# Nicolas-Zamorano/pytorch_fem_solver

Hardware: AMD Instinct MI355X
Metric: Melements/s assembled (global K + f) (higher is better)
Workload: dtype f64

## Files before the change

### pytorch_fem_solver_amd/basis/engine.py

```python

from __future__ import annotations

import ctypes
import math
import os
from ctypes import c_void_p

import numpy as np
import torch

from .. import _native
from ..sparse import CSRMatrix


class NoDeviceError(RuntimeError):
    pass


def _is_block(u):
    return u is not None and u.dim() == 2 and u.shape[1] > 1


def _compute_device(home: torch.device) -> torch.device:
    if home.type == "cuda":
# ... 155 lines not shown
                c_void_p(coords.ctypes.data), c_void_p(rowptr.ctypes.data),
                c_void_p(colind.ctypes.data), own_cap, vert_cap, flags, ctypes.byref(handle),
                ctypes.byref(n_priority),
            )
        )
    try:
        layout = np.zeros(32, dtype=np.int64)
        _native.check(lib.tfem_ring_plan_sizes(handle, c_void_p(layout.ctypes.data)))
        blob = np.empty(int(layout[12]), dtype=np.uint8)
        _native.check(lib.tfem_ring_plan_pack(handle, c_void_p(blob.ctypes.data)))
    finally:
        lib.tfem_ring_plan_destroy(handle)
    plan = unpack_ring_plan(blob, layout)
    plan["n_priority"] = int(n_priority.value)
    return plan


def unpack_ring_plan(blob, layout):
    z = [int(x) for x in layout]

    def view(i, dtype, count):
        return np.frombuffer(blob, dtype=dtype, count=count, offset=z[8 + i])

    return {
        "blob": blob,
        "layout": np.ascontiguousarray(layout, dtype=np.int64),
        "n_tiles": z[0],
        "slots": z[6],
        "words": z[7],
        "chunked": bool(z[13]),
        "desc": view(0, np.int32, 20 * z[0]),
        "rows": view(1, np.uint32, z[7] * z[1]),
        "rowstart": view(2, np.int32, z[1]),
        "vert_gid": view(3, np.int32, z[2]),
        "row_ecodes": np.frombuffer(blob, dtype=np.uint32, count=((12 * z[6] + 31) // 32) * z[1], offset=z[15]),
        "tile_elems": np.frombuffer(blob, dtype=np.int32, count=z[19], offset=z[16]),
        "tile_tverts": np.frombuffer(blob, dtype=np.uint32, count=z[21], offset=z[20]),
        "long_rows": np.frombuffer(blob, dtype=np.uint32, count=24 * z[23], offset=z[22]),
        "elems_staged": bool(z[18]),
        "chain_order": np.frombuffer(blob, dtype=np.int32, count=z[0], offset=z[24]),
        "chain_len": z[25],
        "hand_in": np.frombuffer(blob, dtype=np.uint16, count=z[1], offset=z[26]),
        "max_n_tv": z[27],
        "n_runs": z[28],
        "runs": np.frombuffer(blob, dtype=np.int32, count=(z[28] + 1 if z[28] > 0 else 0), offset=z[30]),
    }


def p2_plan_host(conn_dof, n_verts, n_dofs, coords, rowptr, colind):
    lib = _native.load()
    conn = np.ascontiguousarray(np.asarray(conn_dof).astype(np.int32)).reshape(-1, 6)
    coords = np.ascontiguousarray(np.asarray(coords, dtype=np.float64)).reshape(-1, 2)
    rowptr = np.ascontiguousarray(np.asarray(rowptr, dtype=np.int64))
    colind = np.ascontiguousarray(np.asarray(colind, dtype=np.int32))
    handle = c_void_p()
    _native.check(
        lib.tfem_p2_plan_create(
            c_void_p(conn.ctypes.data), conn.shape[0], int(n_verts), int(n_dofs),
            c_void_p(coords.ctypes.data), c_void_p(rowptr.ctypes.data),
            c_void_p(colind.ctypes.data), ctypes.byref(handle),
        )
    )
    try:
        layout = np.zeros(24, dtype=np.int64)
        _native.check(lib.tfem_p2_plan_sizes(handle, c_void_p(layout.ctypes.data)))
        blob = np.zeros(int(layout[16]), dtype=np.uint8)
        _native.check(lib.tfem_p2_plan_pack(handle, c_void_p(blob.ctypes.data)))
    finally:
# ... 424 lines not shown
            return {"priority": (0, p), "rest": (p, n - p), "all": (0, n)}[which]
        except KeyError:
            raise ValueError(f"tiles: {which!r} is not 'priority', 'rest' or 'all'") from None

    def _resident_source_workgroups(self):
        cus = 256
        if self.device.type == "cuda":
            cus = int(torch.cuda.get_device_properties(self.device).multi_processor_count)
        try:
            reserve = max(0, int(os.environ.get("TFEM_RINGS_RESERVE_CUS", "0") or 0))
        except ValueError:
            reserve = 0
        return (max(8, cus - 8 * reserve) * 4 // 8) * 8

    def ring_plan(self):
        if self._rings is None:
            self._rings = False
            if self.kernel in ("auto", "rings") and self._p1_plan_eligible():
                self.csr_structure()
                rowptr, colind = self._csr_host
                wgs_given = os.environ.get("TFEM_RING_WGS")
                if wgs_given is None:
                    os.environ["TFEM_RING_WGS"] = str(self._resident_source_workgroups())
                try:
                    plan = ring_plan_host(
                        self._conn_host_np(), self.n_dofs, self._coords_host_np(), rowptr, colind,
                        priority=self._priority_vertices, pattern=self._pattern,
                    )
                except NotImplementedError:
                    plan = None
                finally:
                    if wgs_given is None:
                        os.environ.pop("TFEM_RING_WGS", None)
                    if self._pattern is not None:
                        self._pattern.release()
                        self._pattern = None
                if plan is not None:
                    step = np.diff(plan["rowstart"].astype(np.int64))
                    n_runs = 1 + int(np.count_nonzero((step <= 0) | (step > 16)))
                    self._rings = {
                        "blob": torch.from_numpy(plan["blob"]).to(self.device),
                        "layout": plan["layout"],
                        "chunked": plan["chunked"],
                        "elems_staged": plan["elems_staged"],
                        "has_tverts": int(plan["layout"][21]) > 0 or int(plan["layout"][19]) == 0,
                        "fq_ok": bool(plan["elems_staged"]) and int(plan["layout"][23]) == 0,
                        "rows_per_run": plan["rowstart"].size / n_runs,
                        "n_tiles": plan["n_tiles"],
                        "n_priority": plan["n_priority"],
                    }
            if self._rings is False and self.kernel == "rings":
                raise NotImplementedError("the ring-plan kernel does not apply to this basis")
        return self._rings or None

    def p2_plan(self):
        if self._p2rows is None:
# ... 967 lines not shown
```

### pytorch_fem_solver_amd/csrc/tfem_rings.hip

```cpp
#include <cmath>

#include "tfem_rings_kernel.hpp"

namespace tfem {

template <typename T, bool MASS>
__global__ __launch_bounds__(kRingBlock) void k_p1_long_rows(const T *coords, const unsigned char *plan,
                                                             unsigned off_long, int n_long, T *vals, T stiff_w,
                                                             T mass_d, T mass_o) {
  RingLongSlot<T> s;
  ring_long_slot<T, MASS, false>(coords, plan, off_long, n_long, stiff_w, mass_o, nullptr, s);
  if (!s.slot) return;
  T *out = vals + s.rec[1];
  out[int((s.rec[19 + s.i / 8] >> (4 * (s.i % 8))) & 15u)] = s.entry;
  if (s.i == 0) out[s.dpos] = ring_diag<T, MASS>(s.sum, s.dsum, mass_d, mass_o);
}

struct RingLaunch {
  const void *coords;
  int quad_order;
  double alpha, beta;
  const unsigned char *plan;
  const int64_t *layout;
  int64_t n_verts, nnz;
// ... 190 lines not shown
    a.u_first = int(t_first);
    if (z[28] > 0 && (t_first != 0 || t_count != z[0]))
      return fail(TFEM_ERR_UNSUPPORTED, "tile ranges need a plan built with flagged vertices (its blocks break between the ranges)");
    if (z[28] > 0) {
      a.n_runs = int(z[28]);
      a.off_runs = unsigned(z[30]);
    }
  } else {
    a.off_desc += 80u * unsigned(t_first);
  }
  const bool mass = L.beta != 0.0;
  const int slots = int(z[6]);
  a.lds_elem = load ? int(z[17]) : 0;
  const size_t lds = size_t(4 * a.lds_vert) * sizeof(T) +
                     (kmat ? size_t(kRingWaves) * size_t(64 * (slots + 1) + 2) * sizeof(T) : 0) +
                     (src ? size_t(3 * (a.lds_vert + 2)) * sizeof(T)
                          : load ? size_t(3 * a.lds_elem + 4) * sizeof(T) : 0);
  const bool chunk = z[13] != 0;
  a.plain_stores = !load;
  if (const char *v = std::getenv("TFEM_RINGS_STORES")) a.plain_stores = std::strcmp(v, "plain") == 0;
  const bool wide = src && ring_src_wide(L.source);
  const bool separable = src && ring_src_route<T>(z, L.coords, tables.nq, L.source) == 2;
  if (separable) ring_separable_weights<T>(L.source, a.qsym);
  void *kernel = pick_ring_kernel<T>(slots, mass, chunk, load ? tables.nq : 0, src, kmat, wide, separable);
  if (!kernel) return fail(TFEM_ERR_UNSUPPORTED, "Integration order not implemented");
  int per_cu = 0;
  st = resident_per_cu(kernel, kRingBlock, lds, &per_cu);
  if (st != TFEM_OK) return st;
  const int deal = a.xcd_interleave > 0 ? a.xcd_interleave : 1;
  int per = int((t_count + 8 * deal - 1) / (8 * deal)) * deal;
  if (src) {
    const int64_t first_block = t_first / a.chain_len, last_block = (t_first + t_count - 1) / a.chain_len;
    per = int((last_block - first_block + 1 + 7) / 8);
    if (a.n_runs > 0) per = (a.n_runs + 7) / 8;
  }
  if (L.blocks_per_cu > 0 && L.blocks_per_cu < per_cu) per_cu = L.blocks_per_cu;
  int cus = device_cu_count();
  if (const char *v = std::getenv("TFEM_RINGS_RESERVE_CUS")) cus = std::max(8, cus - 8 * std::max(0, std::atoi(v)));
  const int blocks = std::min(per * 8, (cus * per_cu / 8) * 8);
  const dim3 grid{unsigned(blocks)}, block{unsigned(kRingBlock)};
  void *params[] = {&a};
  hipError_t e = hipLaunchKernel(kernel, grid, block, params, lds, L.stream);
  if (e != hipSuccess) return fail(TFEM_ERR_HIP, "ring kernel launch: %s", hipGetErrorString(e));
  if (kmat && z[23] > 0) {
    const dim3 lgrid{unsigned((16 * z[23] + kRingBlock - 1) / kRingBlock)};
    if (mass)
// ... 117 lines not shown
```

### pytorch_fem_solver_amd/csrc/tfem_rings_host.cpp

```cpp
#include <algorithm>
#include <cmath>
#include <cstdlib>
#include <cstring>
#include <memory>
#include <numeric>
#include <vector>
#include <chrono>
#include <cstdio>

#include "tfem_common.hpp"
#include "tfem_threads.hpp"

namespace tfem {

constexpr int kRingDescStride = 20;
constexpr int kRingLayoutLen = 32;
constexpr int kRingElemCap = 768;
constexpr int kRingElemRuns = 8;
constexpr int kRingHaloCapHost = 256;

struct RingPlan {
  int slots = 7, words = 4;
  std::vector<int32_t> desc;
  std::vector<uint32_t> rows;
  std::vector<int32_t> rowstart;
  std::vector<int32_t> tile_elems;
  std::vector<uint32_t> row_ecodes;
  std::vector<uint32_t> tile_tverts;
  std::vector<uint32_t> long_rows;
  int32_t max_n_elem = 0;
  bool elems_staged = true;
  std::vector<int32_t> vert_gid;
  int32_t max_n_vert = 0, max_n_own = 0, max_row_len = 0, max_n_halo = 0;
  int64_t n_tiles = 0;
  bool chunked = false;
  bool long_mode = false;
  int64_t n_priority = 0;
  std::vector<int32_t> chain_order;
  std::vector<uint16_t> hand_in;
  int32_t chain_len = 1;
  std::vector<int32_t> runs;
  int32_t chain_wgs = 1024;
  int32_t max_n_tv = 0;
};

namespace {

inline uint64_t ring_spread_bits(uint64_t x) {
  x &= 0xFFFFFFFFull;
  x = (x | (x << 16)) & 0x0000FFFF0000FFFFull;
  x = (x | (x << 8)) & 0x00FF00FF00FF00FFull;
  x = (x | (x << 4)) & 0x0F0F0F0F0F0F0F0Full;
  x = (x | (x << 2)) & 0x3333333333333333ull;
  x = (x | (x << 1)) & 0x5555555555555555ull;
  return x;
}

struct Fan {
  int k = 0;
  int32_t nb[16];
  int flag[16];
  int32_t elem[16];
  int loc[16];
};

// ... 495 lines not shown
  std::vector<uint8_t> starts(size_t(n_tiles), 0);
  if (runs.empty()) {
    for (int64_t u = 0; u < n_tiles; u += len) starts[size_t(u)] = 1;
    if (n_priority > 0 && n_priority < n_tiles) starts[size_t(n_priority)] = 1;
    return starts;
  }
  for (size_t w = 0; w + 1 < runs.size(); ++w)
    if (runs[w] < runs[w + 1]) starts[size_t(runs[w])] = 1;
  return starts;
}

void chain_pass(const std::vector<TileSpec> &specs, RingPlan &plan) {
  const int64_t n_tiles = plan.n_tiles;
  plan.chain_order.resize(size_t(n_tiles));
  std::iota(plan.chain_order.begin(), plan.chain_order.end(), 0);
  auto by_curve = [&](int32_t x, int32_t y) { return specs[size_t(x)].curve_rank < specs[size_t(y)].curve_rank; };
  std::sort(plan.chain_order.begin(), plan.chain_order.begin() + plan.n_priority, by_curve);
  std::sort(plan.chain_order.begin() + plan.n_priority, plan.chain_order.end(), by_curve);
  const int len = pick_chain_len(n_tiles);
  plan.chain_len = len;
  plan.chain_wgs = 1024;
  if (const char *v = std::getenv("TFEM_RING_WGS")) plan.chain_wgs = std::max(8, std::atoi(v));
  plan.runs.clear();
  bool use_runs = plan.n_priority == 0;
  if (const char *v = std::getenv("TFEM_RING_RUNS")) use_runs = use_runs && std::atoi(v) != 0;
  if (use_runs) plan.runs = chain_runs(n_tiles, plan.chain_wgs);
  const std::vector<uint8_t> starts = chain_block_starts(n_tiles, len, plan.runs, plan.n_priority);
  plan.hand_in.assign(plan.rowstart.size(), uint16_t(0xFFFF));
  std::vector<int64_t> block_first;
  for (int64_t u = 0; u < n_tiles; ++u)
    if (starts[size_t(u)]) block_first.push_back(u);
  block_first.push_back(n_tiles);
  const int64_t n_blocks = int64_t(block_first.size()) - 1;
  std::vector<std::vector<uint32_t>> kept(static_cast<size_t>(n_tiles));
  int32_t *desc = plan.desc.data();
  auto elem_id = [&](const int32_t *d, int32_t j) {
    const int32_t *te = plan.tile_elems.data() + d[16];
    if (!d[18]) return te[j];
    int32_t id = te[0] + j;
    for (int r = 1; r < kRingElemRuns; ++r)
      if (j >= te[kRingElemRuns + r - 1]) id = te[r] + (j - te[kRingElemRuns + r - 1]);
    return id;
  };
  parallel_for(n_blocks, [&](int64_t b0, int64_t b1, int) {
    TileMap prev(16384), cur(16384), prev_local(2048);
    for (int64_t b = b0; b < b1; ++b) {
// ... 287 lines not shown
          return fail(TFEM_ERR_UNSUPPORTED, "vertex %d alone exceeds the tile capacity", u);
        break;
      }
      for (int32_t w : fresh) vert_stamp[size_t(w)] = tile;
      n_local += int(fresh.size());
      spec.owned.push_back(u);
      ++cursor;
    }
    std::sort(spec.owned.begin(), spec.owned.end());
    for (int w = 0; w < 5; ++w) spec.wave_start[w] = std::min<int32_t>(64 * w, int32_t(spec.owned.size()));
    spec.curve_rank = tile;
    specs.push_back(std::move(spec));
    ++tile;
  }
  lap("greedy tiling along the curve");
  priority_first(specs);
  const int st = emit_plan(conn, adj_ptr_data, adj_data, rowptr, colind, elem_ranges, specs, plan);
  lap("emitting tiles");
  if (st == TFEM_OK) chain_pass(specs, plan);
  lap("chain order, element tables");
  return st;
}

void ring_layout(const RingPlan &p, int64_t layout[kRingLayoutLen]) {
  std::memset(layout, 0, sizeof(int64_t) * kRingLayoutLen);
  layout[0] = p.n_tiles;
  layout[1] = int64_t(p.rowstart.size());
  layout[2] = int64_t(p.vert_gid.size());
  layout[3] = p.max_n_vert;
  layout[4] = p.max_n_own;
  layout[5] = p.max_row_len;
  layout[6] = p.slots;
  layout[7] = p.words;
  const int64_t bytes[11] = {int64_t(p.desc.size()) * 4, int64_t(p.rows.size()) * 4,
                             int64_t(p.rowstart.size()) * 4, int64_t(p.vert_gid.size()) * 4,
                             int64_t(p.row_ecodes.size()) * 4, int64_t(p.tile_elems.size()) * 4,
                             int64_t(p.tile_tverts.size()) * 4, int64_t(p.long_rows.size()) * 4,
                             int64_t(p.chain_order.size()) * 4, int64_t(p.hand_in.size()) * 2,
                             int64_t(p.runs.size()) * 4};
  const int slot_of[11] = {8, 9, 10, 11, 15, 16, 20, 22, 24, 26, 30};
  int64_t off = 0;
  for (int i = 0; i < 11; ++i) {
    layout[slot_of[i]] = off;
    off += (bytes[i] + 15) & ~int64_t(15);
  }
  layout[12] = off + 64;
  layout[17] = p.max_n_elem;
  layout[18] = p.elems_staged ? 1 : 0;
  layout[19] = int64_t(p.tile_elems.size());
  layout[21] = int64_t(p.tile_tverts.size());
  layout[23] = int64_t(p.long_rows.size() / 24);
  layout[13] = p.chunked ? 1 : 0;
  layout[14] = p.max_n_halo;
  layout[25] = p.chain_len;
  layout[27] = p.max_n_tv;
  layout[28] = p.runs.empty() ? -1 : p.chain_wgs;
}

}
}

namespace tfem {
namespace {
int ring_plan_build(const void *conn_host, int idx_bytes, int64_t n_elems, int64_t n_verts,
                    const double *coords_host, const int64_t *rowptr_host, const int32_t *colind_host,
                    int own_cap, int vert_cap, const uint8_t *vertex_priority_host, const int64_t *inc_ptr,
                    int32_t *inc, void **plan_out, int64_t *n_priority_tiles) {
  if (!plan_out) return fail(TFEM_ERR_INVALID_ARGUMENT, "plan_out is NULL");
// ... 75 lines not shown
  auto *out = static_cast<unsigned char *>(blob_host);
  struct Part { int64_t off; const void *src; int64_t bytes; };
  const Part parts[11] = {
      {layout[8], p->desc.data(), int64_t(p->desc.size()) * 4},
      {layout[9], p->rows.data(), int64_t(p->rows.size()) * 4},
      {layout[10], p->rowstart.data(), int64_t(p->rowstart.size()) * 4},
      {layout[11], p->vert_gid.data(), int64_t(p->vert_gid.size()) * 4},
      {layout[15], p->row_ecodes.data(), int64_t(p->row_ecodes.size()) * 4},
      {layout[16], p->tile_elems.data(), int64_t(p->tile_elems.size()) * 4},
      {layout[20], p->tile_tverts.data(), int64_t(p->tile_tverts.size()) * 4},
      {layout[22], p->long_rows.data(), int64_t(p->long_rows.size()) * 4},
      {layout[24], p->chain_order.data(), int64_t(p->chain_order.size()) * 4},
      {layout[26], p->hand_in.data(), int64_t(p->hand_in.size()) * 2},
      {layout[30], p->runs.data(), int64_t(p->runs.size()) * 4},
  };
  for (const Part &part : parts) {
    const int64_t padded = (part.bytes + 15) & ~int64_t(15);
    std::memset(out + part.off + part.bytes, 0, size_t(padded - part.bytes));
    if (part.bytes == 0) continue;
    parallel_for(part.bytes, [&](int64_t b, int64_t e, int) {
      std::memcpy(out + part.off + b, static_cast<const unsigned char *>(part.src) + b, size_t(e - b));
    }, 1 << 20);
  }
  std::memset(out + layout[12] - 64, 0, 64);
  return TFEM_OK;
}

int tfem_ring_plan_vouch_coords(int64_t *plan_layout_host, const void *coords, double max_abs_coord) {
  if (!plan_layout_host) return tfem::fail(TFEM_ERR_INVALID_ARGUMENT, "plan_layout_host is NULL");
  int64_t bits = 0, array = 0;
  if (coords && max_abs_coord >= 0.0 && std::isfinite(max_abs_coord)) {
    std::memcpy(&bits, &max_abs_coord, sizeof(bits));
    array = int64_t(reinterpret_cast<uintptr_t>(coords));
  }
  plan_layout_host[29] = array;
  plan_layout_host[31] = bits;
  return TFEM_OK;
}

void tfem_ring_plan_destroy(void *plan_handle) { delete static_cast<tfem::RingPlan *>(plan_handle); }

}
```

### pytorch_fem_solver_amd/csrc/tfem_rings_kernel.hpp

```cpp
#pragma once

#include <hip/hip_runtime.h>

#include <algorithm>
#include <cstdlib>
#include <cstring>
#include <type_traits>

#include "tfem_common.hpp"
#include "tfem_rowkit.hpp"
#include "tfem_source.hpp"

#pragma clang fp contract(fast)

namespace tfem {

constexpr int kRingBlock = 256;
constexpr int kRingWaves = kRingBlock / 64;
constexpr int kRingVertCap = 1024;

template <typename T>
struct RingArgs {
  const T *coords;
  const unsigned char *plan;
// ... 379 lines not shown
}

template <int SLOTS>
__device__ __forceinline__ void ring_load_rec(ring_rsrc_t r, unsigned byte, RingRec<SLOTS> &rec) {
  const ru32x4 v = __builtin_amdgcn_raw_buffer_load_b128(r, byte, 0, kStreamLoadNT);
  rec.w[0] = v.x;
  rec.w[1] = v.y;
  rec.w[2] = v.z;
  rec.w[3] = v.w;
  if constexpr (SLOTS == 15) {
    const ru32x4 u = __builtin_amdgcn_raw_buffer_load_b128(r, byte + 16u, 0, kStreamLoadNT);
    rec.w[4] = u.x;
    rec.w[5] = u.y;
    rec.w[6] = u.z;
    rec.w[7] = u.w;
  }
}

struct RingDesc {
  int vert_off, n_vert, row_off, n_own, row0, row1, gid0, rs0, elem_off, n_elem, elem_mode, tvert_off;
  int n_tv;
};
constexpr int kRingElemRuns = 8;

template <bool CHUNK>
__device__ __forceinline__ RingDesc ring_desc(const unsigned char *plan, unsigned off_desc, int tile,
                                              int wave) {
  ring_const_i32 d = (ring_const_i32)(uintptr_t)(plan + off_desc + 80u * unsigned(tile));
  RingDesc r{d[0], d[1], d[2], d[7], d[3 + wave], d[4 + wave], 0, 0, d[16], d[17], d[18] & 0xFF, d[19], d[18] >> 8};
  if (CHUNK) {
    r.gid0 = d[8 + wave];
    r.rs0 = d[12 + wave];
  }
  return r;
}

constexpr int kRingHaloCap = kRingBlock;
constexpr int kRingElemPerLane = 3;

__device__ __forceinline__ void ring_lds_barrier() {
  asm volatile("s_waitcnt lgkmcnt(0)\n\ts_barrier" ::: "memory");
}

constexpr int kFqLoadNT = 0;
template <typename T, int QL>
__device__ __forceinline__ void ring_load_fq(ring_rsrc_t r, unsigned byte, T (&v)[QL > 0 ? QL : 1]) {
// ... 89 lines not shown
    }
  };
  ring_rsrc_t r_coords = ring_rsrc(a.coords, a.coords_bytes);
  ring_rsrc_t r_plan = ring_rsrc(a.plan, a.plan_bytes);
  ring_rsrc_t r_vals = ring_rsrc(a.vals, a.vals_bytes);
  const ring_rsrc_t r_fq = ring_rsrc(a.fq, a.fq_bytes);
  ring_rsrc_t r_fout = ring_rsrc(a.fout, a.fout_bytes);
  constexpr unsigned kRecBytes = unsigned(4 * RingRec<SLOTS>::kWords);
  constexpr unsigned kNone = 0x3FFFFFFu;
  auto tile_rsrc = [&](unsigned off, int first, int count, int size) {
    const unsigned at = off + unsigned(first * size);
    const int room = int(plan_room - at), want = count * size;
    const int fits = want < room ? want : room;
    return ring_rsrc(plan_at + at, unsigned(fits > 0 ? fits : 0));
  };
  auto run_rsrc = [&](T *vals, unsigned vals_room, int first, int count) {
    const int at = first > 0 ? first : 0;
    const int room = int(vals_room / unsigned(sizeof(T))) - at;
    const int fits = count < room ? count : room;
    return ring_rsrc(reinterpret_cast<unsigned char *>(vals) + unsigned(at) * unsigned(sizeof(T)),
                     unsigned(fits > 0 ? fits : 0) * unsigned(sizeof(T)));
  };
  const unsigned lane_b2 = unsigned(lane) * 2u, lane_b4 = unsigned(lane) * 4u, lane_b16 = unsigned(lane) * 16u;
  if (FQ && tid < 4)
    gtab[3 * a.lds_elem + tid] = T(0);
  const int acc_stride = a.lds_vert + 2;
  T *accs = gtab;
  if (SRC)
    for (int i = tid; i < 3 * acc_stride; i += kRingBlock) accs[i] = T(0);

  SrcLanes<T> prog;
  if constexpr (SRC && !SEP) prog = src_load_lanes<T>(src_in_kernarg<T>(__builtin_offsetof(RingArgs<T>, src)));
  int sep_flags = 0;
  if constexpr (SEP) sep_flags = src_separable_flags<T>(src_in_kernarg<T>(__builtin_offsetof(RingArgs<T>, src)));
  RingRec<SLOTS> rec, rec_ld;
  uint32_t se[FQ ? kEW : 1], se_ld[FQ ? kEW : 1];
  unsigned eid[FQ ? kRingElemPerLane : 1], eid_ld[FQ ? kRingElemPerLane : 1];
  T fqe_ld[FQ ? kRingElemPerLane : 1][QL > 0 ? QL : 1];
  unsigned tev[SRC ? kRingElemPerLane : 1], tev_ld[SRC ? kRingElemPerLane : 1];
  unsigned gid_row = 0;
  int rowstart = 0, rowstart_ld = 0;
  unsigned gid_own = 0, gid_halo = 0;
  unsigned gid_own_ld = 0, gid_halo_ld = 0;
  T own_ld[2], halo_ld[2];
  unsigned hin = 0xFFFFu, hin_ld = 0xFFFFu;

// ... 161 lines not shown
        const T base = src_fma<T>(qs[0], f4[0], qs[1] * ((f4[1] + f4[2]) + f4[3]));
        share[j][0] = det * src_fma<T>(qs[2], f4[3], base);
        share[j][1] = det * src_fma<T>(qs[2], f4[1], base);
        share[j][2] = det * src_fma<T>(qs[2], f4[2], base);
      } else {
        T fw[QL > 0 ? QL : 1];
#pragma unroll
        for (int q = 0; q < QL; ++q) fw[q] = fv[j * (QL > 0 ? QL : 1) + q] * hwq[q];
#pragma unroll
        for (int i = 0; i < 3; ++i) {
          T g = T(0);
#pragma unroll
          for (int q = 0; q < QL; ++q) g = g + fw[q] * lamq[i][q];
          share[j][i] = det * g;
        }
      }
    }
#pragma unroll
    for (int j = 0; j < kNE; ++j)
#pragma unroll
      for (int i = 0; i < 3; ++i) asm volatile("" : "+v"(share[j][i]));
#pragma unroll
    for (int j = 0; j < kNE; ++j) {
      if (vtid + j * kRingBlock < d.n_tv) {
#pragma unroll
        for (int i = 0; i < 3; ++i) add_share((codes[j] >> (10 * i)) & 0x3FFu, acc, share[j][i]);
      }
    }
  };
  auto compute_g = [&](const RingDesc &d, const unsigned (&tv)[SRC ? kRingElemPerLane : 1], const T *xyc,
                       T *acc, int rot) {
    const int vwave = (wave + rot) & (kRingWaves - 1);
    const int vtid = (vwave << 6) + lane;
    const int rounds = (d.n_tv - vwave * 64 + kRingBlock - 1) / kRingBlock;
    if (rounds <= 0) return;
    if constexpr (SRC == 2) {
      if (rounds >= 3)
        compute_g_wide(std::integral_constant<int, 3>{}, d, tv, xyc, acc, vtid);
      else
        compute_g_wide(std::integral_constant<int, 2>{}, d, tv, xyc, acc, vtid);
    } else if constexpr (SRC == 1) {
      unsigned codes[kRingElemPerLane];
#pragma unroll
      for (int j = 0; j < kRingElemPerLane; ++j) codes[j] = tv[SRC ? j : 0];
#pragma unroll 1
      for (int j = 0; j < kRingElemPerLane; ++j) {
        if (j >= rounds) break;
        const int l = vtid + j * kRingBlock;
        const unsigned code = codes[0];
#pragma unroll
        for (int r = 0; r + 1 < kRingElemPerLane; ++r) codes[r] = codes[r + 1];
        T x0, y0, x1, y1, x2, y2;
        lds_xy(xyc, code & 0x3FFu, x0, y0);
        lds_xy(xyc, (code >> 10) & 0x3FFu, x1, y1);
// ... 62 lines not shown
      dst[2 * r + 1] = own_ld[1];
    }
    const int h = d.n_own + tid;
    if (h < d.n_vert) {
      dst[2 * h] = halo_ld[0];
      dst[2 * h + 1] = halo_ld[1];
    }
  };
  auto load_xy_lds = [&](const RingDesc &d, unsigned g_own, unsigned g_halo, T *dst) {
    if constexpr (kCoordsToLds) {
      typedef __attribute__((address_space(3))) void *lds_ptr;
      if constexpr (kTileDesc && CHUNK) {
        if (lane < d.row1 - d.row0)
          __builtin_amdgcn_raw_ptr_buffer_load_lds(r_coords, (lds_ptr)(dst + 2 * d.row0), 16,
                                                   (unsigned(lane) << 4) + unsigned(d.gid0) * 16u, 0, 0, 0);
      } else if (d.row0 + lane < d.row1)
        __builtin_amdgcn_raw_ptr_buffer_load_lds(r_coords, (lds_ptr)(dst + 2 * d.row0), 16, g_own * 16u, 0, 0, 0);
      if (d.n_own + tid < d.n_vert)
        __builtin_amdgcn_raw_ptr_buffer_load_lds(r_coords, (lds_ptr)(dst + 2 * (d.n_own + 64 * wave)), 16,
                                                 g_halo * 16u, 0, 0, 0);
    }
  };

  int t_c = tile_at(0);
  if (t_c < 0) return;
  int t_n = tile_at(1), t_nn = tile_at(2);
  RingDesc dc = ring_desc<CHUNK>(a.plan, a.off_desc, t_c, wave);
  RingDesc dn = ring_desc<CHUNK>(a.plan, a.off_desc, t_n >= 0 ? t_n : t_c, wave);
  RingDesc dnn = ring_desc<CHUNK>(a.plan, a.off_desc, t_nn >= 0 ? t_nn : t_c, wave);
  load_ids(dc, gid_own, gid_halo);
  load_eids(dc, eid);
  __builtin_amdgcn_s_waitcnt(0x0F70);
  load_tile(dc, gid_own, gid_halo);
  load_xy_lds(dc, gid_own, gid_halo, xy);
  load_fq(dc, eid);
  load_tverts(dc, tev_ld, 0);
  if (t_n >= 0) {
    load_ids(dn, gid_own_ld, gid_halo_ld);
    load_eids(dn, eid_ld);
  }
  __builtin_amdgcn_s_waitcnt(0x0F70);
  park(dc, xy);
  park_g(dc, gtab);
  rec = rec_ld;
  hin = hin_ld;
  rowstart = rowstart_ld;
  gid_row = gid_own;
#pragma unroll
  for (int i = 0; i < (FQ ? kEW : 1); ++i) se[i] = se_ld[i];
#pragma unroll
  for (int j = 0; j < (FQ ? kRingElemPerLane : 1); ++j) eid[j] = eid_ld[j];
#pragma unroll
  for (int j = 0; j < (SRC ? kRingElemPerLane : 1); ++j) tev[j] = tev_ld[j];
  gid_own = gid_own_ld;
  gid_halo = gid_halo_ld;
  __syncthreads();

  int cur = 0;
  int a_cur = 0, a_prev = 2, a_next = 1;
  for (int k = 0;; ++k) {
    if (SRC) {
      switch ((k + int(blockIdx.x >> kRingPrioShift)) & 3) {
        case 0: __builtin_amdgcn_s_setprio(0); break;
        case 1: __builtin_amdgcn_s_setprio(1); break;
        case 2: __builtin_amdgcn_s_setprio(2); break;
        default: __builtin_amdgcn_s_setprio(3); break;
      }
    }
    auto phase_a = [&]() {
      if (t_n >= 0) {
        load_tile(dn, gid_own, gid_halo);
        load_fq(dn, eid);
        load_tverts(dn, tev_ld, k + 1);
        if (t_nn >= 0) {
          load_ids(dnn, gid_own_ld, gid_halo_ld);
          load_eids(dnn, eid_ld);
        }
      }
    };
    if (SRC) {
      if (t_n >= 0) load_xy_lds(dn, gid_own, gid_halo, xy + (cur ^ 1) * 2 * a.lds_vert);
      compute_g(dc, tev, xy + cur * 2 * a.lds_vert, accs + a_cur * acc_stride, k);
      if constexpr (SEP) {
        typedef const RingArgs<T> __attribute__((address_space(4))) *ring_kernargs;
        const ring_kernargs ka = (ring_kernargs)src_kernarg_table<char>(0);
        r_coords = ring_rsrc(ka->coords, ka->coords_bytes);
        plan_at = ka->plan;
        plan_room = ka->plan_bytes;
        vals_at = ka->vals;
        vals_room = ka->vals_bytes;
        plain_now = ka->plain_stores;
        r_vals = ring_rsrc(vals_at, vals_room);
        r_fout = ring_rsrc(ka->fout, ka->fout_bytes);
      }
    }
    phase_a();
    T off[SLOTS + 1], diag, sdets[SLOTS];
    constexpr int kBandSlots = (SLOTS > kRingBand && kRingBand > 0) ? kRingBand : (SLOTS == 7 && SRC ? 6 : SLOTS);
    const bool banded = kBandSlots < SLOTS && __builtin_amdgcn_ballot_w64(rec.k() > kBandSlots) == 0;
    bool regular = false;
    const int my_row = dc.row0 + lane;
    const uint32_t lv = unsigned(my_row < dc.row1 ? my_row : 0);
    if constexpr (SLOTS == 7 && SRC) {
      const bool mine = ((rec.w[2] >> 10) & 0x3FFFu) == 0x555u && rec.k() == 6;
// ... 96 lines not shown
        __builtin_amdgcn_raw_buffer_store_b64(__builtin_bit_cast(ru32x2, facc), r_fout, byte, 0, kStreamNT);
      else
        __builtin_amdgcn_raw_buffer_store_b32(__builtin_bit_cast(unsigned, facc), r_fout, byte, 0, kStreamNT);
    }
    if (t_n < 0) break;
    rec = rec_ld;
    hin = hin_ld;
    rowstart = rowstart_ld;
    gid_row = gid_own;
#pragma unroll
    for (int i = 0; i < (FQ ? kEW : 1); ++i) se[i] = se_ld[i];
#pragma unroll
    for (int j = 0; j < (FQ ? kRingElemPerLane : 1); ++j) eid[j] = eid_ld[j];
#pragma unroll
    for (int j = 0; j < (SRC ? kRingElemPerLane : 1); ++j) tev[j] = tev_ld[j];
    gid_own = gid_own_ld;
    gid_halo = gid_halo_ld;
    {
      const int t = a_prev;
      a_prev = a_cur;
      a_cur = a_next;
      a_next = t;
    }
    ring_lds_barrier();
    t_c = t_n;
    dc = dn;
    t_n = t_nn;
    dn = dnn;
    t_nn = tile_at(k + 3);
    if (t_nn >= 0) dnn = ring_desc<CHUNK>(plan_now(), a.off_desc, t_nn, wave);
    cur ^= 1;
  }
}

template <typename T>
void *pick_ring_src_kernel(int slots, bool mass, bool chunk, int nq, bool kmat, bool wide, bool separable);
inline bool ring_src_runs_wide(int nq, bool wide) { return wide && nq <= 4; }

template <typename T>
static int ring_args_init(const TriTables &tables, const int64_t *z, const void *coords, const unsigned char *plan,
                   int64_t n_verts, double alpha, double beta, RingArgs<T> &a) {
  if (z[0] < 0 || z[4] > kRingBlock || z[3] > kRingVertCap || z[4] > z[3] || z[14] > kRingHaloCap ||
      !((z[6] == 7 && z[7] == 4) || (z[6] == 15 && z[7] == 8)) || (z[5] > z[6] + 1 && z[23] == 0) || z[5] > 16)
    return fail(TFEM_ERR_INVALID_ARGUMENT, "ring plan exceeds the kernel's capacities");
  const int64_t extents[2] = {n_verts * 2 * int64_t(sizeof(T)), z[12]};
  const int st = check_extents("ring kernel", extents, 2);
// ... 26 lines not shown
```

Measured before the change: 78190.

## Precompute per-wave tile walk records on host for separable source ring kernel

```diff
diff --git a/pytorch_fem_solver_amd/basis/engine.py b/pytorch_fem_solver_amd/basis/engine.py
--- a/pytorch_fem_solver_amd/basis/engine.py
+++ b/pytorch_fem_solver_amd/basis/engine.py
@@ -201,6 +201,8 @@
     def view(i, dtype, count):
         return np.frombuffer(blob, dtype=dtype, count=count, offset=z[8 + i])
 
+    has_walk = (bool(z[13]) and z[6] == 7 and z[28] > 0
+                and ((z[30] + 4 * (z[28] + 1) + 63) & ~63) + 256 * z[0] + 64 <= z[12])
     return {
         "blob": blob,
         "layout": np.ascontiguousarray(layout, dtype=np.int64),
@@ -223,6 +225,8 @@
         "max_n_tv": z[27],
         "n_runs": z[28],
         "runs": np.frombuffer(blob, dtype=np.int32, count=(z[28] + 1 if z[28] > 0 else 0), offset=z[30]),
+        "walk": np.frombuffer(blob, dtype=np.int32, count=(64 * z[0] if has_walk else 0),
+                              offset=(((z[30] + 4 * (z[28] + 1) + 63) & ~63) if has_walk else 0)).reshape(-1, 4, 16),
     }
 
 
@@ -693,6 +697,9 @@
                 wgs_given = os.environ.get("TFEM_RING_WGS")
                 if wgs_given is None:
                     os.environ["TFEM_RING_WGS"] = str(self._resident_source_workgroups())
+                walk_given = os.environ.get("TFEM_RING_WALK")
+                if walk_given is None:
+                    os.environ["TFEM_RING_WALK"] = "1"
                 try:
                     plan = ring_plan_host(
                         self._conn_host_np(), self.n_dofs, self._coords_host_np(), rowptr, colind,
@@ -703,6 +710,8 @@
                 finally:
                     if wgs_given is None:
                         os.environ.pop("TFEM_RING_WGS", None)
+                    if walk_given is None:
+                        os.environ.pop("TFEM_RING_WALK", None)
                     if self._pattern is not None:
                         self._pattern.release()
                         self._pattern = None
diff --git a/pytorch_fem_solver_amd/csrc/tfem_rings.hip b/pytorch_fem_solver_amd/csrc/tfem_rings.hip
--- a/pytorch_fem_solver_amd/csrc/tfem_rings.hip
+++ b/pytorch_fem_solver_amd/csrc/tfem_rings.hip
@@ -236,6 +236,11 @@
   const bool wide = src && ring_src_wide(L.source);
   const bool separable = src && ring_src_route<T>(z, L.coords, tables.nq, L.source) == 2;
   if (separable) ring_separable_weights<T>(L.source, a.qsym);
+  if (src) a.off_telems = 0;
+  if (separable && chunk && slots == 7 && a.n_runs > 0) {
+    const int64_t walk_at = (z[30] + 4 * (z[28] + 1) + 63) & ~int64_t(63);
+    if (walk_at + 256 * z[0] + 64 <= z[12]) a.off_telems = unsigned(walk_at);
+  }
   void *kernel = pick_ring_kernel<T>(slots, mass, chunk, load ? tables.nq : 0, src, kmat, wide, separable);
   if (!kernel) return fail(TFEM_ERR_UNSUPPORTED, "Integration order not implemented");
   int per_cu = 0;
diff --git a/pytorch_fem_solver_amd/csrc/tfem_rings_host.cpp b/pytorch_fem_solver_amd/csrc/tfem_rings_host.cpp
--- a/pytorch_fem_solver_amd/csrc/tfem_rings_host.cpp
+++ b/pytorch_fem_solver_amd/csrc/tfem_rings_host.cpp
@@ -41,6 +41,7 @@
   int32_t chain_len = 1;
   std::vector<int32_t> runs;
   int32_t chain_wgs = 1024;
+  bool with_walk = false;
   int32_t max_n_tv = 0;
 };
 
@@ -582,6 +583,7 @@
   plan.chain_wgs = 1024;
   if (const char *v = std::getenv("TFEM_RING_WGS")) plan.chain_wgs = std::max(8, std::atoi(v));
   plan.runs.clear();
+  if (const char *v = std::getenv("TFEM_RING_WALK")) plan.with_walk = v[0] == '1';
   bool use_runs = plan.n_priority == 0;
   if (const char *v = std::getenv("TFEM_RING_RUNS")) use_runs = use_runs && std::atoi(v) != 0;
   if (use_runs) plan.runs = chain_runs(n_tiles, plan.chain_wgs);
@@ -915,6 +917,43 @@
   return st;
 }
 
+constexpr int64_t kRingWalkBytes = 64;
+inline bool ring_has_walk(const RingPlan &p) { return p.with_walk && p.chunked && p.slots == 7 && !p.runs.empty(); }
+inline int64_t ring_walk_offset(int64_t off_runs, int64_t n_runs) { return (off_runs + 4 * (n_runs + 1) + 63) & ~int64_t(63); }
+
+void ring_walk_fill(const RingPlan &p, const int64_t *layout, int32_t *out) {
+  const int64_t n_runs = int64_t(p.runs.size()) - 1;
+  parallel_for(n_runs, [&](int64_t b, int64_t e, int) {
+    for (int64_t r = b; r < e; ++r)
+      for (int64_t u = p.runs[size_t(r)]; u < p.runs[size_t(r) + 1]; ++u) {
+        const int32_t *d = p.desc.data() + size_t(p.chain_order[size_t(u)]) * kRingDescStride;
+        const int64_t k = u - p.runs[size_t(r)];
+        for (int w = 0; w < 4; ++w) {
+          int32_t *rec = out + (size_t(u) * 4 + size_t(w)) * 16;
+          auto stream = [&](int at, int64_t section, int64_t first, int64_t count, int64_t size) {
+            rec[at] = int32_t(count > 0 ? section + first * size : section);
+            rec[at + 1] = int32_t(count > 0 ? count * size : 0);
+          };
+          const int64_t row0 = d[3 + w], rows = d[4 + w] - d[3 + w];
+          stream(0, layout[9], d[2] + row0, rows, 4 * p.words);
+          stream(2, layout[26], d[2] + row0, rows, 2);
+          const int64_t first_e = ((w + k) & 3) << 6, left = (d[18] >> 8) - first_e;
+          stream(4, layout[20], d[19] + first_e, left, 4);
+          rec[6] = int32_t(left);
+          rec[7] = int32_t(left > 0 ? (left + 255) / 256 : 0);
+          rec[8] = d[8 + w];
+          rec[9] = d[12 + w];
+          rec[10] = int32_t(row0);
+          rec[11] = int32_t(rows);
+          const int64_t halo0 = d[7] + 64 * w;
+          stream(12, layout[11], d[0] + halo0, d[1] - halo0, 4);
+          rec[14] = int32_t(halo0);
+          rec[15] = u + 1 == p.runs[size_t(r) + 1] ? 1 : 0;
+        }
+      }
+  }, 4);
+}
+
 void ring_layout(const RingPlan &p, int64_t layout[kRingLayoutLen]) {
   std::memset(layout, 0, sizeof(int64_t) * kRingLayoutLen);
   layout[0] = p.n_tiles;
@@ -937,6 +976,7 @@
     layout[slot_of[i]] = off;
     off += (bytes[i] + 15) & ~int64_t(15);
   }
+  if (ring_has_walk(p)) off = ring_walk_offset(layout[30], int64_t(p.runs.size()) - 1) + p.n_tiles * 4 * kRingWalkBytes;
   layout[12] = off + 64;
   layout[17] = p.max_n_elem;
   layout[18] = p.elems_staged ? 1 : 0;
@@ -1058,6 +1098,12 @@
       std::memcpy(out + part.off + b, static_cast<const unsigned char *>(part.src) + b, size_t(e - b));
     }, 1 << 20);
   }
+  if (ring_has_walk(*p)) {
+    const int64_t runs_end = layout[30] + ((int64_t(p->runs.size()) * 4 + 15) & ~int64_t(15));
+    const int64_t at = ring_walk_offset(layout[30], int64_t(p->runs.size()) - 1);
+    std::memset(out + runs_end, 0, size_t(at - runs_end));
+    ring_walk_fill(*p, layout, reinterpret_cast<int32_t *>(out + at));
+  }
   std::memset(out + layout[12] - 64, 0, 64);
   return TFEM_OK;
 }
diff --git a/pytorch_fem_solver_amd/csrc/tfem_rings_kernel.hpp b/pytorch_fem_solver_amd/csrc/tfem_rings_kernel.hpp
--- a/pytorch_fem_solver_amd/csrc/tfem_rings_kernel.hpp
+++ b/pytorch_fem_solver_amd/csrc/tfem_rings_kernel.hpp
@@ -425,6 +425,14 @@
   int n_tv;
 };
 constexpr int kRingElemRuns = 8;
+
+typedef int ring_walk_t __attribute__((ext_vector_type(16)));
+typedef int ring_walk_half_t __attribute__((ext_vector_type(8)));
+typedef int ring_walk_halo_t __attribute__((ext_vector_type(4)));
+enum : int {
+  kWalkRecOff = 0, kWalkRecBytes, kWalkHinOff, kWalkHinBytes, kWalkTvOff, kWalkTvBytes, kWalkTvLeft, kWalkRounds,
+  kWalkGid0, kWalkRs0, kWalkRow0, kWalkRows, kWalkHaloOff, kWalkHaloBytes, kWalkHaloSlot, kWalkLast
+};
 
 template <bool CHUNK>
 __device__ __forceinline__ RingDesc ring_desc(const unsigned char *plan, unsigned off_desc, int tile,
@@ -560,6 +568,94 @@
                      unsigned(fits > 0 ? fits : 0) * unsigned(sizeof(T)));
   };
   const unsigned lane_b2 = unsigned(lane) * 2u, lane_b4 = unsigned(lane) * 4u, lane_b16 = unsigned(lane) * 16u;
+  constexpr bool kWalk = kTileDesc && CHUNK && SLOTS == 7;
+  int n_gid0 = 0, n_rs0 = 0, n_row0 = 0, n_rows = 0, n_hbytes = 0, n_hslot = 0;
+  int hnn_off = 0, hnn_bytes = 0, hnn_last = 0, cur_left = 0, cur_rounds = 0;
+  unsigned wpos = 0, wpos_n = 0;
+  auto walking = [&]() {
+    unsigned at = a.off_telems;
+    asm volatile("" : "+s"(at));
+    return at != 0u;
+  };
+  auto walk_set_next = [&](const ring_walk_t &w) {
+    n_gid0 = w[kWalkGid0];
+    n_rs0 = w[kWalkRs0];
+    n_row0 = w[kWalkRow0];
+    n_rows = w[kWalkRows];
+    n_hbytes = w[kWalkHaloBytes];
+    n_hslot = w[kWalkHaloSlot];
+  };
+  auto walk_load_next = [&](unsigned at) {
+    typedef int pair_t __attribute__((ext_vector_type(2)));
+    typedef const pair_t __attribute__((address_space(4))) *pair_ptr;
+    const pair_t g = *(pair_ptr)(uintptr_t)(plan_now() + at + 4u * unsigned(kWalkGid0));
+    const pair_t r = *(pair_ptr)(uintptr_t)(plan_now() + at + 4u * unsigned(kWalkRow0));
+    const pair_t h = *(pair_ptr)(uintptr_t)(plan_now() + at + 4u * unsigned(kWalkHaloBytes));
+    n_gid0 = g[0];
+    n_rs0 = g[1];
+    n_row0 = r[0];
+    n_rows = r[1];
+    n_hbytes = h[0];
+    n_hslot = h[1];
+  };
+  auto walk_load = [&](unsigned at) {
+    typedef const ring_walk_t __attribute__((address_space(4))) *walk_ptr;
+    return *(walk_ptr)(uintptr_t)(plan_now() + at);
+  };
+  auto walk_load_half = [&](unsigned at) {
+    typedef const ring_walk_half_t __attribute__((address_space(4))) *half_ptr;
+    return *(half_ptr)(uintptr_t)(plan_now() + at);
+  };
+  auto walk_first = [&](const ring_walk_t &w) { return __builtin_shufflevector(w, w, 0, 1, 2, 3, 4, 5, 6, 7); };
+  auto walk_load_halo = [&](unsigned at) {
+    typedef const ring_walk_halo_t __attribute__((address_space(4))) *halo_ptr;
+    const ring_walk_halo_t h = *(halo_ptr)(uintptr_t)(plan_now() + at + 4u * unsigned(kWalkHaloOff));
+    hnn_off = h[0];
+    hnn_bytes = h[1];
+    hnn_last = h[3];
+  };
+  auto walk_next_run = [&]() {
+    for (;;) {
+      run += int(gridDim.x);
+      if (run >= a.n_runs) return false;
+      ring_const_i32 first = (ring_const_i32)(uintptr_t)(plan_now() + a.off_runs);
+      const int u0 = first[run];
+      if (u0 < first[run + 1]) {
+        wpos = a.off_telems + 64u * unsigned(wave) + 256u * unsigned(u0);
+        return true;
+      }
+    }
+  };
+  auto walk_step = [&](int last) {
+    if (last) return walk_next_run() ? 0 : -1;
+    wpos += 256u;
+    return 0;
+  };
+  auto walk_of_desc = [&](const RingDesc &d, int rot) {
+    ring_walk_t w = {};
+    auto stream = [&](int at, unsigned off, int first, int count, int size) {
+      const unsigned from = off + unsigned(first * size);
+      const int room = int(plan_room - from), want = count * size;
+      const int fits = want < room ? want : room;
+      w[at] = int(from);
+      w[at + 1] = fits > 0 ? fits : 0;
+    };
+    const int first = d.row_off + d.row0, n = d.row1 - d.row0;
+    stream(kWalkRecOff, a.off_rows, first, n, int(kRecBytes));
+    stream(kWalkHinOff, a.off_hin, first, n, 2);
+    const int first_e = ((wave + rot) & (kRingWaves - 1)) << 6;
+    stream(kWalkTvOff, a.off_tverts, d.tvert_off + first_e, d.n_tv - first_e, 4);
+    w[kWalkTvLeft] = d.n_tv - first_e;
+    w[kWalkRounds] = (d.n_tv - first_e + kRingBlock - 1) / kRingBlock;
+    w[kWalkGid0] = d.gid0;
+    w[kWalkRs0] = d.rs0;
+    w[kWalkRow0] = d.row0;
+    w[kWalkRows] = n;
+    stream(kWalkHaloOff, a.off_gid, d.vert_off + d.n_own + 64 * wave, d.n_vert - d.n_own - 64 * wave, 4);
+    w[kWalkHaloSlot] = d.n_own + 64 * wave;
+    return w;
+  };
+  auto walk_rsrc = [&](int off, int bytes) { return ring_rsrc(plan_at + unsigned(off), unsigned(bytes)); };
   if (FQ && tid < 4)
     gtab[3 * a.lds_elem + tid] = T(0);
   const int acc_stride = a.lds_vert + 2;
@@ -767,7 +863,12 @@
       for (int i = 0; i < 3; ++i) asm volatile("" : "+v"(share[j][i]));
 #pragma unroll
     for (int j = 0; j < kNE; ++j) {
-      if (vtid + j * kRingBlock < d.n_tv) {
+      bool mine;
+      if constexpr (kWalk)
+        mine = vtid + j * kRingBlock < cur_left;
+      else
+        mine = vtid + j * kRingBlock < d.n_tv;
+      if (mine) {
 #pragma unroll
         for (int i = 0; i < 3; ++i) add_share((codes[j] >> (10 * i)) & 0x3FFu, acc, share[j][i]);
       }
@@ -775,6 +876,14 @@
   };
   auto compute_g = [&](const RingDesc &d, const unsigned (&tv)[SRC ? kRingElemPerLane : 1], const T *xyc,
                        T *acc, int rot) {
+    if constexpr (kWalk) {
+      if (cur_rounds <= 0) return;
+      if (cur_rounds >= 3)
+        compute_g_wide(std::integral_constant<int, 3>{}, d, tv, xyc, acc, lane);
+      else
+        compute_g_wide(std::integral_constant<int, 2>{}, d, tv, xyc, acc, lane);
+      return;
+    }
     const int vwave = (wave + rot) & (kRingWaves - 1);
     const int vtid = (vwave << 6) + lane;
     const int rounds = (d.n_tv - vwave * 64 + kRingBlock - 1) / kRingBlock;
@@ -883,22 +992,116 @@
     }
   };
 
-  int t_c = tile_at(0);
-  if (t_c < 0) return;
-  int t_n = tile_at(1), t_nn = tile_at(2);
-  RingDesc dc = ring_desc<CHUNK>(a.plan, a.off_desc, t_c, wave);
-  RingDesc dn = ring_desc<CHUNK>(a.plan, a.off_desc, t_n >= 0 ? t_n : t_c, wave);
-  RingDesc dnn = ring_desc<CHUNK>(a.plan, a.off_desc, t_nn >= 0 ? t_nn : t_c, wave);
-  load_ids(dc, gid_own, gid_halo);
-  load_eids(dc, eid);
-  __builtin_amdgcn_s_waitcnt(0x0F70);
-  load_tile(dc, gid_own, gid_halo);
-  load_xy_lds(dc, gid_own, gid_halo, xy);
-  load_fq(dc, eid);
-  load_tverts(dc, tev_ld, 0);
-  if (t_n >= 0) {
-    load_ids(dn, gid_own_ld, gid_halo_ld);
-    load_eids(dn, eid_ld);
+  auto load_ids_walk = [&](int off, int bytes, unsigned &g_halo) {
+    g_halo = __builtin_amdgcn_raw_buffer_load_b32(walk_rsrc(off, bytes), lane_b4, 0, 0);
+  };
+  auto load_tile_walk = [&](const ring_walk_half_t &w) {
+    ring_load_rec<SLOTS>(walk_rsrc(w[kWalkRecOff], w[kWalkRecBytes]), lane_b16 * (kRecBytes / 16u), rec_ld);
+    hin_ld = __builtin_amdgcn_raw_buffer_load_b16(walk_rsrc(w[kWalkHinOff], w[kWalkHinBytes]), lane_b2, 0, 0);
+  };
+  auto load_tverts_walk = [&](const ring_walk_half_t &w, unsigned (&tv)[SRC ? kRingElemPerLane : 1]) {
+    const ring_rsrc_t r_tv = walk_rsrc(w[kWalkTvOff], w[kWalkTvBytes]);
+#pragma unroll
+    for (int j = 0; j < kRingElemPerLane; ++j)
+      tv[SRC ? j : 0] =
+          __builtin_amdgcn_raw_buffer_load_b32(r_tv, lane_b4 + unsigned(4 * j * kRingBlock), 0, kStreamLoadNT);
+  };
+  auto load_xy_lds_walk = [&](unsigned g_halo, T *dst) {
+    typedef __attribute__((address_space(3))) void *lds_ptr;
+    if (lane < n_rows)
+      __builtin_amdgcn_raw_ptr_buffer_load_lds(r_coords, (lds_ptr)(dst + 2 * n_row0), 16,
+                                               (unsigned(lane) << 4) + unsigned(n_gid0) * 16u, 0, 0, 0);
+    if (int(lane_b4) < n_hbytes)
+      __builtin_amdgcn_raw_ptr_buffer_load_lds(r_coords, (lds_ptr)(dst + 2 * n_hslot), 16, g_halo * 16u, 0, 0, 0);
+  };
+  int t_c, t_n, t_nn;
+  auto walk_take = [&](RingDesc &d) {
+    d.row0 = n_row0;
+    d.row1 = n_row0 + n_rows;
+    d.gid0 = n_gid0;
+    d.rs0 = n_rs0;
+  };
+  auto walk_streams = [&](int k1) {
+    if (walking()) return walk_load_half(wpos_n);
+    return walk_first(walk_of_desc(ring_desc<CHUNK>(plan_now(), a.off_desc, t_n, wave), k1));
+  };
+
+  RingDesc dc, dn, dnn;
+  if constexpr (kWalk) {
+    ring_walk_t w0;
+    int halo1_off = 0, halo1_bytes = 0;
+    if (walking()) {
+      if (!walk_next_run()) return;
+      t_c = 0;
+      w0 = walk_load(wpos);
+      t_n = walk_step(w0[kWalkLast]);
+      t_nn = -1;
+      if (t_n >= 0) {
+        wpos_n = wpos;
+        const ring_walk_t w1 = walk_load(wpos);
+        walk_set_next(w1);
+        halo1_off = w1[kWalkHaloOff];
+        halo1_bytes = w1[kWalkHaloBytes];
+        t_nn = walk_step(w1[kWalkLast]);
+      }
+      if (t_nn >= 0) walk_load_halo(wpos);
+    } else {
+      t_c = tile_at(0);
+      if (t_c < 0) return;
+      t_n = tile_at(1);
+      t_nn = tile_at(2);
+      w0 = walk_of_desc(ring_desc<CHUNK>(a.plan, a.off_desc, t_c, wave), 0);
+      if (t_n >= 0) {
+        const ring_walk_t w1 = walk_of_desc(ring_desc<CHUNK>(a.plan, a.off_desc, t_n, wave), 1);
+        walk_set_next(w1);
+        halo1_off = w1[kWalkHaloOff];
+        halo1_bytes = w1[kWalkHaloBytes];
+      }
+      if (t_nn >= 0) {
+        const ring_walk_t w2 = walk_of_desc(ring_desc<CHUNK>(a.plan, a.off_desc, t_nn, wave), 2);
+        hnn_off = w2[kWalkHaloOff];
+        hnn_bytes = w2[kWalkHaloBytes];
+      }
+    }
+    dc = dn = dnn = RingDesc{};
+    load_ids_walk(w0[kWalkHaloOff], w0[kWalkHaloBytes], gid_halo);
+    __builtin_amdgcn_s_waitcnt(0x0F70);
+    load_tile_walk(walk_first(w0));
+    {
+      const int keep[6] = {n_gid0, n_rs0, n_row0, n_rows, n_hbytes, n_hslot};
+      walk_set_next(w0);
+      load_xy_lds_walk(gid_halo, xy);
+      walk_take(dc);
+      n_gid0 = keep[0];
+      n_rs0 = keep[1];
+      n_row0 = keep[2];
+      n_rows = keep[3];
+      n_hbytes = keep[4];
+      n_hslot = keep[5];
+    }
+    load_tverts_walk(walk_first(w0), tev_ld);
+    if (t_n >= 0) load_ids_walk(halo1_off, halo1_bytes, gid_halo_ld);
+    cur_left = w0[kWalkTvLeft];
+    cur_rounds = w0[kWalkRounds];
+  } else {
+    t_c = tile_at(0);
+    if (t_c < 0) return;
+    t_n = tile_at(1);
+    t_nn = tile_at(2);
+    dc = ring_desc<CHUNK>(a.plan, a.off_desc, t_c, wave);
+    dn = ring_desc<CHUNK>(a.plan, a.off_desc, t_n >= 0 ? t_n : t_c, wave);
+    dnn = ring_desc<CHUNK>(a.plan, a.off_desc, t_nn >= 0 ? t_nn : t_c, wave);
+    load_ids(dc, gid_own, gid_halo);
+    load_eids(dc, eid);
+    __builtin_amdgcn_s_waitcnt(0x0F70);
+    load_tile(dc, gid_own, gid_halo);
+    load_xy_lds(dc, gid_own, gid_halo, xy);
+    load_fq(dc, eid);
+    load_tverts(dc, tev_ld, 0);
+    if (t_n >= 0) {
+      load_ids(dn, gid_own_ld, gid_halo_ld);
+      load_eids(dn, eid_ld);
+    }
   }
   __builtin_amdgcn_s_waitcnt(0x0F70);
   park(dc, xy);
@@ -929,6 +1132,17 @@
       }
     }
     auto phase_a = [&]() {
+      if constexpr (kWalk) {
+        if (t_n >= 0) {
+          const ring_walk_half_t ws = walk_streams(k + 1);
+          load_tile_walk(ws);
+          load_tverts_walk(ws, tev_ld);
+          if (t_nn >= 0) load_ids_walk(hnn_off, hnn_bytes, gid_halo_ld);
+          cur_left = ws[kWalkTvLeft];
+          cur_rounds = ws[kWalkRounds];
+        }
+        return;
+      }
       if (t_n >= 0) {
         load_tile(dn, gid_own, gid_halo);
         load_fq(dn, eid);
@@ -940,7 +1154,10 @@
       }
     };
     if (SRC) {
-      if (t_n >= 0) load_xy_lds(dn, gid_own, gid_halo, xy + (cur ^ 1) * 2 * a.lds_vert);
+      if constexpr (kWalk) {
+        if (t_n >= 0) load_xy_lds_walk(gid_halo, xy + (cur ^ 1) * 2 * a.lds_vert);
+      } else if (t_n >= 0)
+        load_xy_lds(dn, gid_own, gid_halo, xy + (cur ^ 1) * 2 * a.lds_vert);
       compute_g(dc, tev, xy + cur * 2 * a.lds_vert, accs + a_cur * acc_stride, k);
       if constexpr (SEP) {
         typedef const RingArgs<T> __attribute__((address_space(4))) *ring_kernargs;
@@ -1083,6 +1300,30 @@
       a_cur = a_next;
       a_next = t;
     }
+    if constexpr (kWalk) {
+      walk_take(dc);
+      t_c = t_n;
+      t_n = t_nn;
+      if (walking()) {
+        if (t_n >= 0) {
+          wpos_n = wpos;
+          walk_load_next(wpos);
+          t_nn = walk_step(hnn_last);
+          if (t_nn >= 0) walk_load_halo(wpos);
+        }
+      } else if (t_n >= 0) {
+        walk_set_next(walk_of_desc(ring_desc<CHUNK>(plan_now(), a.off_desc, t_n, wave), k + 2));
+        t_nn = tile_at(k + 3);
+        if (t_nn >= 0) {
+          const ring_walk_t w2 = walk_of_desc(ring_desc<CHUNK>(plan_now(), a.off_desc, t_nn, wave), 0);
+          hnn_off = w2[kWalkHaloOff];
+          hnn_bytes = w2[kWalkHaloBytes];
+        }
+      }
+      ring_lds_barrier();
+      cur ^= 1;
+      continue;
+    }
     ring_lds_barrier();
     t_c = t_n;
     dc = dn;
```

Measured after the change: 78770 (median of 6 runs). About the same (+0.7%).
